# larskaislaniemi/PyLamp

Hardware: AMD Instinct MI355X
Metric: stokes_heat_mic_cell_updates_per_s (higher is better)
Workload: dtype f64

## Files before the change

pylamp_amd/csrc/pl_mic.h:

```cpp
#pragma once
#include "pl_internal.h"

#define PL_MAX_SCATTER_FIELDS 8
#define PL_MAX_GATHER_FIELDS 8

#define PL_AVG_PRELOG 64
struct PlScatterArgs {
    long long n;
    const double* tz; const double* tx;
    int nf;
    const double* f[PL_MAX_SCATTER_FIELDS];
    int scheme[PL_MAX_SCATTER_FIELDS];
    double z0, hz, x0, hx;
    double rhz, rhx;
    const double* zc; const double* xc;
    int nz, nx;
    int row0, nrows, col0, ncols;
    double* wsum; double* cnt;
    double* acc[PL_MAX_SCATTER_FIELDS];
    const int* cell_start; int ncz, ncx;
    int crow0, ccol0;
    int stag_z, stag_x;
};

// ... 79 lines not shown
    int nz, nx;
    int row0, nrows, col0, ncols;
    const int* cell_start; int ncz, ncx, crow0, ccol0;
    double* accN; double* accC; double* accZ; double* accX;
    long long N;
    int* slow_count; int* slow_list; int slow_cap;
    int dbg;
};
#define PL_SCF_MAX 10
struct PlScatterFinalArgs {
    int nz, nx, nf;
    const double* acc[PL_SCF_MAX]; const double* den[PL_SCF_MAX]; int scheme[PL_SCF_MAX]; double* out[PL_SCF_MAX];
    long long acc_pitch, out_pitch, out_off;
};
int pl_scatter_cells_device(pl_ctx* ctx, PlScatterCellsArgs& a, int variant);
void pl_launch_scatter_finalize_multi(pl_ctx* ctx, const PlScatterFinalArgs& a);

__device__ inline void mic_axis_locate(const double* __restrict__ c, int n, double z, int& ie, double& a) {
    if (z < c[0]) {
        const double h = c[1] - c[0], f = floor((z - c[0]) / h);
        ie = (int)f; a = (z - (c[0] + f * h)) / h;
        return;
    }
    if (z > c[n - 1]) {
        const double h = c[n - 1] - c[n - 2], f = floor((z - c[n - 1]) / h);
        ie = n - 1 + (int)f; a = (z - (c[n - 1] + f * h)) / h;
        return;
    }
    int lo = 0, hi = n - 1;
    while (hi - lo > 1) { const int mid = (lo + hi) >> 1; if (c[mid] <= z) lo = mid; else hi = mid; }
// ... 12 lines not shown
```

pylamp_amd/csrc/pl_mic_cells.hip:

```cpp
#include "pl_internal.h"
#include "pl_mic.h"

#define SC_Q 4
#define SC_NL 16
#define SC_W (SC_NL - 2)
#ifndef SC_ROWS
#define SC_ROWS 32
#endif
#ifndef SC_CAP
#define SC_CAP 320
#endif
#define SC_CAPP (SC_CAP + SC_CAP / 16 + 2)
#ifndef SC_NB
#define SC_NB 2
#endif

__device__ inline int sc_pidx(int o) { return o + (o >> 4); }

template <int CTRL> __device__ inline double sc_dpp(double v) {
    int lo = __double2loint(v), hi = __double2hiint(v);
    lo = __builtin_amdgcn_update_dpp(0, lo, CTRL, 0xf, 0xf, false);
    hi = __builtin_amdgcn_update_dpp(0, hi, CTRL, 0xf, 0xf, false);
    return __hiloint2double(hi, lo);
}
// ... 315 lines not shown
                const int di = cnr & 1, dj = cnr >> 1;
                double w = (dj ? cb : 1.0 - cb) * (di ? ca : 1.0 - ca);
                const bool flat = set == 1 && CEN == 2;
                if (flat) w = 1.0;
                add(base, ie + di, je + dj, w);
                for (int f = 0; f < nfs; f++) {
                    const int fk = set == 0 ? f : (NFN > 1 ? 1 : 0);
                    const double v = set <= 1 ? a.fn[fk][(IMASK >> fk) & 1u ? e : t] : a.fm[IND ? e : t];
                    add(base + (long long)(1 + f) * a.N, ie + di, je + dj, v * w);
                }
            }
        }
    }
}

__global__ __launch_bounds__(256) void k_scatter_finalize_multi(PlScatterFinalArgs a) {
    const int j = blockIdx.x * 64 + threadIdx.x, i = blockIdx.y * 4 + threadIdx.y;
    if (j >= a.nx || i >= a.nz) return;
    const long long o = (long long)i * a.acc_pitch + j, oo = a.out_off + (long long)i * a.out_pitch + j;
    for (int k = 0; k < a.nf; k++) {
        double s = a.acc[k][o];
        const double d = a.den[k][o];
        double r;
        if (a.scheme[k] & PL_AVG_ARITHMETIC) r = s / d;
        else { if (isinf(s)) s = 0.0; r = exp(s / d); }
        a.out[k][oo] = r;
    }
}

void pl_launch_scatter_finalize_multi(pl_ctx* ctx, const PlScatterFinalArgs& a) {
// ... 25 lines not shown
```

pylamp_amd/csrc/pl_step.hip:

```cpp
#include "pl_internal.h"
#include "pl_mic.h"
#include <algorithm>
#include <chrono>
#include <cmath>
#include <limits>

#define NFTRAC 13
enum { TR_RHO = 0, TR_ETA, TR_MRK, TR_TMP, TR_HCD, TR_HCP, TR_RH0, TR_ALP, TR_MAT, TR_ACE, TR_ET0, TR_IHT, TR__ID };
#define GASR 8.31446
#define PL_EPS (1.0 / 1024.0)

constexpr int X0_HIST = 5;
struct PlStepState {
    long long n = 0, cap = 0;
    double* tz = nullptr; double* tx = nullptr;
    double* tz2 = nullptr; double* tx2 = nullptr;
    double* f[NFTRAC] = {nullptr};
    double* vtz = nullptr; double* vtx = nullptr;
    double* tmp[3] = {nullptr, nullptr, nullptr};
    double* partial = nullptr;
    std::vector<double> hpartial;
    double* gcoords = nullptr;
    bool have_newtemp = false, have_solution = false, have_dT = false;
    int n_prev = 0;
    double* x_hist[X0_HIST] = {};
    double dt_hist[X0_HIST + 1] = {};
    double* f2[NFTRAC] = {nullptr};
    int* cell = nullptr; int* dest = nullptr;
    int* orig = nullptr; int* orig2 = nullptr;
    int* cell_count = nullptr; int* cell_start = nullptr; int* block_sums = nullptr;
    int ncz = 0, ncx = 0;
    int crow0 = 0, ccol0 = 0;
    bool sorted = false;
    int* need = nullptr; int* need_off = nullptr;
    int* need_flag = nullptr; int* need_rank = nullptr;
    int* cell_res = nullptr;
    double max_id = -1.0;
    bool max_id_valid = false;
    int sort_cells = 0;
    int* slot = nullptr; int* slot2 = nullptr;
    bool epoch_on = false; int epoch_age = 0;
    long long epoch_len = 0;
    bool lazy_pending = false, lazy_inject = false; long long lazy_n = 0;
    bool cols_undefined = false;
    std::vector<double> gmz, gmx;
    double* flags = nullptr; double* counts_dev = nullptr; int counts_cap = 0;
};

static PlStepState* state_of(pl_ctx* ctx) {
    if (!ctx->step) ctx->step = new PlStepState();
    return (PlStepState*)ctx->step;
}

void pl_step_free(pl_ctx* ctx) {
    PlStepState* s = (PlStepState*)ctx->step;
    if (!s) return;
    for (double* q : {s->tz, s->tx, s->tz2, s->tx2, s->vtz, s->vtx, s->tmp[0], s->tmp[1], s->tmp[2], s->partial, s->gcoords})
        if (q) (void)hipFree(q);
    for (double* q : s->f) if (q) (void)hipFree(q);
    for (double* q : s->f2) if (q) (void)hipFree(q);
    for (double* q : {s->flags, s->counts_dev}) if (q) (void)hipFree(q);
    for (int* q : {s->slot, s->slot2, s->cell, s->dest, s->orig, s->orig2, s->cell_count, s->cell_start, s->block_sums, s->need, s->need_off, s->need_flag, s->need_rank, s->cell_res}) if (q) (void)hipFree(q);
    delete s;
    ctx->step = nullptr;
}

static dim3 grid2d(const PlGeom& g) { return dim3((g.lnx + 63) / 64, (g.lnz + 3) / 4); }
static dim3 grid1d(long long n) { return dim3((unsigned)std::max<long long>((n + 255) / 256, 1)); }

__global__ __launch_bounds__(256) void k_soa_from_aos2(long long m, const double* __restrict__ src, double* __restrict__ a,
                                                       double* __restrict__ b) {
    long long t = (long long)blockIdx.x * blockDim.x + threadIdx.x;
    if (t < m) { a[t] = src[2 * t]; b[t] = src[2 * t + 1]; }
}
__global__ __launch_bounds__(256) void k_aos2_from_soa(long long m, const double* __restrict__ a, const double* __restrict__ b,
                                                       double* __restrict__ dst) {
    long long t = (long long)blockIdx.x * blockDim.x + threadIdx.x;
// ... 43 lines not shown
    const int base = blockIdx.x * 1024 + threadIdx.x * 4;
    int v[4], s = 0;
    for (int k = 0; k < 4; k++) { v[k] = (base + k < m) ? in[base + k] : 0; s += v[k]; }
    sh[threadIdx.x] = s;
    __syncthreads();
    for (int o = 1; o < 256; o <<= 1) {
        int add = (threadIdx.x >= o) ? sh[threadIdx.x - o] : 0;
        __syncthreads();
        sh[threadIdx.x] += add;
        __syncthreads();
    }
    int run = sh[threadIdx.x] - s;
    for (int k = 0; k < 4; k++) { if (base + k < m) out[base + k] = run; run += v[k]; }
    if (threadIdx.x == 255) bsum[blockIdx.x] = sh[255];
}
__global__ void k_scan_sums(int nb, int* __restrict__ bsum) {
    __shared__ int carry;
    if (threadIdx.x == 0) carry = 0;
    __syncthreads();
    for (int b0 = 0; b0 < nb; b0 += 256) {
        __shared__ int sh[256];
        const int k = b0 + threadIdx.x;
        const int v = (k < nb) ? bsum[k] : 0;
        sh[threadIdx.x] = v;
        __syncthreads();
        for (int o = 1; o < 256; o <<= 1) {
            int add = (threadIdx.x >= o) ? sh[threadIdx.x - o] : 0;
            __syncthreads();
            sh[threadIdx.x] += add;
            __syncthreads();
        }
        if (k < nb) bsum[k] = carry + sh[threadIdx.x] - v;
        __syncthreads();
        if (threadIdx.x == 255) carry += sh[255];
        __syncthreads();
    }
}
__global__ __launch_bounds__(256) void k_scan_add(int m, int* __restrict__ out, const int* __restrict__ bsum, int total_slot) {
    const int k = blockIdx.x * 256 + threadIdx.x;
    if (k < m) out[k] += bsum[k / 1024];
    (void)total_slot;
}
__global__ __launch_bounds__(256) void k_cell_place(long long n, const int* __restrict__ cell, const int* __restrict__ start,
                                                    int* __restrict__ fill, int* __restrict__ dest) {
    const long long t = (long long)blockIdx.x * blockDim.x + threadIdx.x;
    const int lane = threadIdx.x & 63;
    const int c = (t < n) ? cell[t] : -1;
    int seg0, len;
    mic_wave_runs(c, lane, seg0, len);
    int base = 0;
// ... 38 lines not shown
    const long long t = (long long)blockIdx.x * blockDim.x + threadIdx.x;
    const int lane = threadIdx.x & 63;
    const int c = (t < n) ? cell[t] : -1;
    int seg0, len;
    mic_wave_runs(c, lane, seg0, len);
    int base = 0;
    if (lane == seg0 && c >= 0) base = atomicAdd(&fill[c], len);
    base = __shfl(base, seg0, 64);
    if (c < 0) return;
    const int d = start[c] + base + (lane - seg0);
    dest[t] = d;
    for (int k = 0; k < a.na; k++) a.out[k][d] = a.in[k][t];
    slot_out[d] = slot_in ? slot_in[t] : (int)t;
}

__global__ __launch_bounds__(256) void k_deficit(int nc, int ncx, int row_lo, int row_hi, const int* __restrict__ start,
                                                 int dens, int dmin, int* __restrict__ need, int* __restrict__ flag) {
    const int c = blockIdx.x * 256 + threadIdx.x;
    if (c > nc) return;
    int v = 0;
    if (c < nc) {
        const int row = c / ncx;
        const int cnt = start[c + 1] - start[c];
        if (row >= row_lo && row < row_hi && cnt < dmin) v = dens - cnt;
    }
    need[c] = v;
    flag[c] = v > 0 ? 1 : 0;
}
__global__ __launch_bounds__(256) void k_max1d(long long n, const double* __restrict__ v, double* __restrict__ part) {
    double m = -INFINITY;
    for (long long t = (long long)blockIdx.x * 256 + threadIdx.x; t < n; t += (long long)gridDim.x * 256) m = fmax(m, v[t]);
    __shared__ double sh[4];
    for (int o = 32; o > 0; o >>= 1) m = fmax(m, __shfl_down(m, o, 64));
    if ((threadIdx.x & 63) == 0) sh[threadIdx.x >> 6] = m;
    __syncthreads();
    if (threadIdx.x == 0) part[blockIdx.x] = fmax(fmax(sh[0], sh[1]), fmax(sh[2], sh[3]));
}
__global__ __launch_bounds__(256) void k_mark_alive(long long n, const int* __restrict__ orig, int* __restrict__ alive) {
    const long long t = (long long)blockIdx.x * blockDim.x + threadIdx.x;
    if (t < n) alive[orig[t]] = 1;
}
__global__ __launch_bounds__(256) void k_remap_orig(long long n, int* __restrict__ orig, const int* __restrict__ rank) {
// ... 211 lines not shown
        *p = nullptr;
        PL_HIP(ctx, hipMalloc((void**)p, (size_t)cap * sizeof(double)));
        return 0;
    };
    for (double** q : {&S->tz, &S->tx, &S->tz2, &S->tx2, &S->vtz, &S->vtx, &S->tmp[0], &S->tmp[1], &S->tmp[2]}) PL_TRY(re(q));
    for (int k = 0; k < NFTRAC; k++) { PL_TRY(re(&S->f[k])); PL_TRY(re(&S->f2[k])); }
    for (int** q : {&S->cell, &S->dest, &S->orig, &S->orig2, &S->slot, &S->slot2}) {
        if (*q) (void)hipFree(*q);
        PL_HIP(ctx, hipMalloc((void**)q, (size_t)cap * sizeof(int)));
    }
    S->cap = cap;
    return 0;
}

static void unpermute(pl_ctx* ctx, PlStepState* S, int na, const double* const* in, double* const* out);
static bool scatter_cells_on() { const char* e = getenv("PYLAMP_SCATTER"); return !(e && atoi(e) == 0); }
static int ensure_current(pl_ctx* ctx, PlStepState* S);
struct SortOpts {
    bool full = false;
    int del_outside = 0; double Lz = 0.0, Lx = 0.0; long long* removed = nullptr;
    const pl_step_config* inject = nullptr; int it = 0; int64_t* ninjected = nullptr;
    bool keys_ready = false;
    bool premigrated = false;
    bool drop_trash = false;
};
static int sort_tracers(pl_ctx* ctx, PlStepState* S, double z0, double hz, double x0, double hx, const SortOpts& o = SortOpts());
static int ensure_coords(pl_ctx* ctx, PlStepState* S) {
    if (S->gcoords) return 0;
    if (S->gmz.empty()) {
        for (int d = 0; d < 2; d++) {
// ... 132 lines not shown
    }
    for (long long t0 = 0; t0 < n; t0 += chunk) {
        long long m = std::min<long long>(chunk, n - t0);
        hipLaunchKernelGGL(k_aos2_from_soa, grid1d(m), dim3(256), 0, ctx->stream, m, S->tz2 + t0, S->tx2 + t0, ctx->stage);
        PL_HIP(ctx, hipMemcpyAsync(out + 2 * t0, ctx->stage, (size_t)m * 2 * sizeof(double), hipMemcpyDeviceToHost, ctx->stream));
        PL_HIP(ctx, hipStreamSynchronize(ctx->stream));
    }
    return 0;
}

struct InjectSorted {
    int nc, ncx, crow0, ccol0;
    const int* start;
    const int* count;
    const int* need; const int* off; const int* rank;
    double* tz; double* tx; double* f[NFTRAC]; double* vtz; double* vtx; int* orig;
    double z0, hz, x0, hx; unsigned long long seed; unsigned step; double id0; int n_old;
    const double* zc; const double* xc;
    int* slot;
    int lazy;
};
__host__ __device__ inline bool tracer_const(int k) { return !(k == TR_RHO || k == TR_ETA || k == TR_TMP); }
__global__ __launch_bounds__(64) void k_inject_sorted(InjectSorted a) {
    const int c = blockIdx.x * 64 + threadIdx.x;
    if (c >= a.nc) return;
    const int m = a.need[c];
    if (m <= 0) return;
    const int t0 = a.start[c], t1 = t0 + a.count[c];
    const int ci = c / a.ncx + a.crow0, cj = c % a.ncx + a.ccol0;
    double mean[NFTRAC];
    for (int k = 0; k < NFTRAC; k++) {
        double sum = 0.0;
        if (a.lazy && (k == TR_RHO || k == TR_ETA)) { mean[k] = 0.0; continue; }
        if (a.slot && tracer_const(k)) for (int t = t0; t < t1; t++) sum += a.f[k][a.slot[t]];
        else for (int t = t0; t < t1; t++) sum += a.f[k][t];
        mean[k] = sum / (double)(t1 - t0);
    }
    for (int q = 0; q < m; q++) {
        const int d = t1 + q;
        const int e = a.slot ? a.n_old + a.off[c] + q : d;
        const unsigned gc = (unsigned)(ci * 65536 + cj);
        const double uz = inj_uniform(a.seed, gc, (unsigned)q, 2 * a.step), ux = inj_uniform(a.seed, gc, (unsigned)q, 2 * a.step + 1);
        a.tz[d] = a.zc ? a.zc[ci] + uz * (a.zc[ci + 1] - a.zc[ci]) : a.z0 + (ci + uz) * a.hz;
        a.tx[d] = a.xc ? a.xc[cj] + ux * (a.xc[cj + 1] - a.xc[cj]) : a.x0 + (cj + ux) * a.hx;
        for (int k = 0; k < NFTRAC; k++) {
            if (a.lazy && (k == TR_RHO || k == TR_ETA)) continue;
            a.f[k][tracer_const(k) ? e : d] = mean[k];
        }
        a.f[TR__ID][e] = a.id0 + a.off[c] + q - (a.rank ? a.rank[c] : 0);
        a.vtz[d] = 0.0; a.vtx[d] = 0.0;
        a.orig[e] = a.n_old + a.off[c] + q;
        if (a.slot) a.slot[d] = e;
    }
}
__global__ __launch_bounds__(64) void k_inject_fix_lazy(int nc, const int* __restrict__ start, const int* __restrict__ count,
                                                        const int* __restrict__ need, double* __restrict__ rho, double* __restrict__ eta) {
    const int c = blockIdx.x * 64 + threadIdx.x;
    if (c >= nc) return;
    const int m = need[c];
    if (m <= 0) return;
    const int t0 = start[c], t1 = t0 + count[c];
    double sr = 0.0, se = 0.0;
    for (int t = t0; t < t1; t++) sr += rho[t];
    for (int t = t0; t < t1; t++) se += eta[t];
    sr /= (double)(t1 - t0); se /= (double)(t1 - t0);
    for (int q = 0; q < m; q++) { rho[t1 + q] = sr; eta[t1 + q] = se; }
}
struct GatherColsArgs { const double* in[5]; double* out[5]; int na; };
__global__ __launch_bounds__(256) void k_gather_cols(long long n, const int* __restrict__ idx, GatherColsArgs a) {
    long long t = (long long)blockIdx.x * blockDim.x + threadIdx.x;
    if (t >= n) return;
    const int s = idx[t];
    for (int k = 0; k < a.na; k++) a.out[k][t] = a.in[k][s];
}
__global__ __launch_bounds__(256) void k_gather_int(long long n, const int* __restrict__ idx, const int* __restrict__ in, int* __restrict__ out) {
    long long t = (long long)blockIdx.x * blockDim.x + threadIdx.x;
    if (t < n) out[t] = in[idx[t]];
}
__global__ __launch_bounds__(256) void k_add_need(int nc, int m, const int* __restrict__ count, const int* __restrict__ need, int* __restrict__ total) {
    const int c = blockIdx.x * 256 + threadIdx.x;
    if (c < m) total[c] = count[c] + (c < nc ? need[c] : 0);
}

static int scan_ints(pl_ctx* ctx, PlStepState* S, int m, const int* in, int* out) {
    const int nb = (m + 1023) / 1024;
    hipLaunchKernelGGL(k_scan_block, dim3(nb), dim3(256), 0, ctx->stream, m, in, out, S->block_sums);
    hipLaunchKernelGGL(k_scan_sums, dim3(1), dim3(256), 0, ctx->stream, nb, S->block_sums);
    hipLaunchKernelGGL(k_scan_add, dim3((m + 255) / 256), dim3(256), 0, ctx->stream, m, out, S->block_sums, 0);
    return 0;
}

static int epoch_length() { const char* e = getenv("PYLAMP_EPOCH"); return e ? atoi(e) : 64; }
static int flush_lazy(pl_ctx* ctx, PlStepState* S) {
    if (!S->lazy_pending) return 0;
    S->lazy_pending = false;
    if (S->lazy_n > 0) {
        PermArgs pa{}; pa.na = 4;
        pa.in[0] = S->f2[TR_RHO]; pa.out[0] = S->f[TR_RHO]; pa.in[1] = S->f2[TR_ETA]; pa.out[1] = S->f[TR_ETA];
        pa.in[2] = S->tmp[0]; pa.out[2] = S->vtz; pa.in[3] = S->tmp[1]; pa.out[3] = S->vtx;
        hipLaunchKernelGGL(k_permute, grid1d(S->lazy_n), dim3(256), 0, ctx->stream, S->lazy_n, S->dest, pa);
    }
    if (S->lazy_inject)
        hipLaunchKernelGGL(k_inject_fix_lazy, dim3((S->sort_cells + 63) / 64), dim3(64), 0, ctx->stream, S->sort_cells, S->cell_start, S->cell_res,
                           S->need, S->f[TR_RHO], S->f[TR_ETA]);
    PL_HIP(ctx, hipGetLastError());
    return 0;
}
static int relayout(pl_ctx* ctx, PlStepState* S) {
    if (!S->epoch_on) return 0;
    S->epoch_on = false; S->epoch_age = 0;
    const long long n = S->n;
    if (n <= 0) return 0;
    int cols[NFTRAC], nc = 0;
    for (int k = 0; k < NFTRAC; k++) if (tracer_const(k)) cols[nc++] = k;
    for (int k0 = 0; k0 < nc; k0 += 5) {
        GatherColsArgs ga{}; ga.na = std::min(5, nc - k0);
        for (int k = 0; k < ga.na; k++) { ga.in[k] = S->f[cols[k0 + k]]; ga.out[k] = S->f2[cols[k0 + k]]; }
        hipLaunchKernelGGL(k_gather_cols, grid1d(n), dim3(256), 0, ctx->stream, n, S->slot, ga);
    }
// ... 16 lines not shown
    const PlGeom& g = ctx->geom.d;
    const int ncz = (g.gi0 + g.lnz >= g.nz) ? g.lnz - 1 : g.lnz;
    const int ncx = (g.gj0 + g.lnx >= g.nx) ? g.lnx - 1 : g.lnx;
    const int nc = ncz * ncx, m = nc + 10;
    S->crow0 = g.gi0; S->ccol0 = g.gj0;
    long long n = S->n;
    if (n >= (1LL << 31)) return pl_fail(ctx, "sort_tracers: more than 2^31 tracers per GPU");
    const bool epoch_ok = !o.full && epoch_length() > 0 && (ctx->nranks == 1 || o.premigrated) && !o.del_outside && ctx->geom.uniform && scatter_cells_on();
    if (!epoch_ok) PL_TRY(ensure_current(ctx, S));
    else {
        PL_TRY(flush_lazy(ctx, S));
        if (S->epoch_on && S->epoch_age >= epoch_length()) PL_TRY(relayout(ctx, S));
    }
    if (!S->cell_count || S->ncz != ncz || S->ncx != ncx) {
        if (o.keys_ready) return pl_fail(ctx, "sort_tracers: sort keys announced for another sort grid (internal error)");
        for (int** q : {&S->cell_count, &S->cell_start, &S->block_sums, &S->need, &S->need_off, &S->need_flag, &S->need_rank, &S->cell_res}) {
            if (*q) (void)hipFree(*q);
            *q = nullptr;
        }
        const int nb = (m + 1023) / 1024;
        for (int** q : {&S->cell_count, &S->cell_start, &S->need, &S->need_off, &S->need_flag, &S->need_rank, &S->cell_res})
            PL_HIP(ctx, hipMalloc((void**)q, (size_t)m * sizeof(int)));
        PL_HIP(ctx, hipMalloc((void**)&S->block_sums, (size_t)(nb + 1) * sizeof(int)));
        S->ncz = ncz; S->ncx = ncx;
    }
    S->sort_cells = nc;
    if (!o.keys_ready) {
        PL_HIP(ctx, hipMemsetAsync(S->cell_count, 0, (size_t)m * sizeof(int), ctx->stream));
        hipLaunchKernelGGL(k_cell_count, grid1d(n), dim3(256), 0, ctx->stream, n, S->tz, S->tx, z0, hz, x0, hx, coords_z(ctx, S, 0),
                           coords_x(ctx, S, 0), ncz, ncx, S->crow0, S->ccol0, g.nz - 1, g.nx - 1, S->cell, S->cell_count, o.del_outside, o.Lz, o.Lx);
    }
    long long ninj = 0; int ndef = 0;
    double id0 = 0.0; bool strict = false;
    const bool inj = o.inject && o.inject->tracdens_min > 0 && o.inject->tracdens > 0;
    if (inj) {
        const pl_step_config* cfg = o.inject;
        scan_ints(ctx, S, m, S->cell_count, S->cell_res);
        hipLaunchKernelGGL(k_deficit, dim3((nc + 1 + 255) / 256), dim3(256), 0, ctx->stream, nc, ncx, 0, ncz, S->cell_res, cfg->tracdens,
                           cfg->tracdens_min, S->need, S->need_flag);
        scan_ints(ctx, S, nc + 1, S->need, S->need_off);
        scan_ints(ctx, S, nc + 1, S->need_flag, S->need_rank);
        int h2[2] = {0, 0};
        PL_HIP(ctx, hipMemcpyAsync(&h2[0], S->need_off + nc, sizeof(int), hipMemcpyDeviceToHost, ctx->stream));
        PL_HIP(ctx, hipMemcpyAsync(&h2[1], S->need_rank + nc, sizeof(int), hipMemcpyDeviceToHost, ctx->stream));
        PL_HIP(ctx, hipStreamSynchronize(ctx->stream));
        ninj = h2[0]; ndef = h2[1];
        const int R = ctx->nranks;
        std::vector<double> cnt((size_t)2 * R, 0.0);
        cnt[2 * ctx->rank] = (double)ninj; cnt[2 * ctx->rank + 1] = ndef;
        if (R > 1) {
            PL_TRY(step_counts(ctx, S, 2 * R));
            hipLaunchKernelGGL(k_counts_from_ints, dim3(1), dim3(64), 0, ctx->stream, 1, (const int*)(S->need_off + nc), 0, S->counts_dev, 2 * ctx->rank);
            hipLaunchKernelGGL(k_counts_from_ints, dim3(1), dim3(64), 0, ctx->stream, 1, (const int*)(S->need_rank + nc), 0, S->counts_dev, 2 * ctx->rank + 1);
            PL_TRY(pl_comm_allreduce_dev(ctx, S->counts_dev, 2 * R, 0));
            PL_HIP(ctx, hipMemcpyAsync(cnt.data(), S->counts_dev, cnt.size() * sizeof(double), hipMemcpyDeviceToHost, ctx->stream));
            PL_HIP(ctx, hipStreamSynchronize(ctx->stream));
// ... 18 lines not shown
                    PL_HIP(ctx, hipStreamSynchronize(ctx->stream));
                    for (int k = 0; k < nbm; k++) mx[0] = std::fmax(mx[0], S->hpartial[k]);
                }
                PL_TRY(pl_allreduce_host(ctx, mx, 1, 2));
                S->max_id = mx[0]; S->max_id_valid = true;
            }
            strict = cfg->inject_unique_ids == 0;
            id0 = strict ? S->max_id + before - def_before : S->max_id + 1.0 + before;
            S->max_id += strict ? total - def_total : total;
        }
        if (ninj > 0) {
            const long long used = std::max(n, (epoch_ok && S->epoch_on) ? S->epoch_len : n);
            PL_TRY(grow_tracers(ctx, S, used + ninj, used));
        }
    }
    if (ninj > 0) {
        hipLaunchKernelGGL(k_add_need, dim3((m + 255) / 256), dim3(256), 0, ctx->stream, nc, m, S->cell_count, S->need, S->cell_res);
        scan_ints(ctx, S, m, S->cell_res, S->cell_start);
        PL_HIP(ctx, hipMemcpyAsync(S->cell_res, S->cell_count, (size_t)m * sizeof(int), hipMemcpyDeviceToDevice, ctx->stream));
    } else {
        scan_ints(ctx, S, m, S->cell_count, S->cell_start);
    }
    PL_HIP(ctx, hipMemsetAsync(S->cell_count, 0, (size_t)m * sizeof(int), ctx->stream));
    if (n > 0 && epoch_ok) {
        PermArgs pa{}; pa.na = 3;
        pa.in[0] = S->tz; pa.out[0] = S->tz2; pa.in[1] = S->tx; pa.out[1] = S->tx2; pa.in[2] = S->f[TR_TMP]; pa.out[2] = S->f2[TR_TMP];
        hipLaunchKernelGGL(k_place_permute, grid1d(n), dim3(256), 0, ctx->stream, n, S->cell, S->cell_start, S->cell_count, S->dest, pa,
                           S->epoch_on ? (const int*)S->slot : (const int*)nullptr, S->slot2);
        std::swap(S->tz, S->tz2); std::swap(S->tx, S->tx2);
        std::swap(S->vtz, S->tmp[0]); std::swap(S->vtx, S->tmp[1]);
        std::swap(S->slot, S->slot2);
        for (int k : {(int)TR_TMP, (int)TR_RHO, (int)TR_ETA}) std::swap(S->f[k], S->f2[k]);
    } else if (n > 0) {
        hipLaunchKernelGGL(k_cell_place, grid1d(n), dim3(256), 0, ctx->stream, n, S->cell, S->cell_start, S->cell_count, S->dest);
        const double* src[17]; double* dst[17];
        src[0] = S->tz; dst[0] = S->tz2; src[1] = S->tx; dst[1] = S->tx2;
// ... 6 lines not shown
        }
        hipLaunchKernelGGL(k_permute_int, grid1d(n), dim3(256), 0, ctx->stream, n, S->dest, S->orig, S->orig2);
        std::swap(S->tz, S->tz2); std::swap(S->tx, S->tx2); std::swap(S->orig, S->orig2);
        std::swap(S->vtz, S->tmp[0]); std::swap(S->vtx, S->tmp[1]);
        for (int k = 0; k < NFTRAC; k++) std::swap(S->f[k], S->f2[k]);
    }
    if (epoch_ok) {
        if (!S->epoch_on) S->epoch_len = n;
        S->epoch_age = S->epoch_on ? S->epoch_age + 1 : 1; S->epoch_on = true;
        S->lazy_pending = true; S->lazy_n = n; S->lazy_inject = ninj > 0;
    }
    if (ninj > 0) {
        InjectSorted a{};
        a.nc = nc; a.ncx = ncx; a.crow0 = S->crow0; a.ccol0 = S->ccol0; a.start = S->cell_start; a.count = S->cell_res;
        a.need = S->need; a.off = S->need_off; a.rank = strict ? S->need_rank : nullptr;
        a.tz = S->tz; a.tx = S->tx; for (int k = 0; k < NFTRAC; k++) a.f[k] = S->f[k];
        a.vtz = S->vtz; a.vtx = S->vtx; a.orig = S->orig;
        a.slot = epoch_ok ? S->slot : nullptr; a.lazy = epoch_ok ? 1 : 0;
        a.z0 = z0; a.hz = hz; a.x0 = x0; a.hx = hx; a.seed = o.inject->inject_seed; a.step = (unsigned)o.it; a.id0 = id0;
        a.n_old = (int)(epoch_ok ? S->epoch_len : n);
        if (epoch_ok) S->epoch_len += ninj;
        a.zc = coords_z(ctx, S, 0); a.xc = coords_x(ctx, S, 0);
        hipLaunchKernelGGL(k_inject_sorted, dim3((nc + 63) / 64), dim3(64), 0, ctx->stream, a);
        S->n = n + ninj;
    }
    if (o.ninjected) *o.ninjected = ninj;
    PL_HIP(ctx, hipGetLastError());
    if (o.removed) *o.removed = 0;
    if (o.drop_trash) {
        int keep = 0;
        PL_HIP(ctx, hipMemcpyAsync(&keep, S->cell_start + nc + 8, sizeof(int), hipMemcpyDeviceToHost, ctx->stream));
        PL_HIP(ctx, hipStreamSynchronize(ctx->stream));
        S->n = keep;
    }
    if (o.del_outside && n > 0) {
        int h[2] = {0, 0};
        PL_HIP(ctx, hipMemcpyAsync(h, S->cell_start + nc + 8, 2 * sizeof(int), hipMemcpyDeviceToHost, ctx->stream));
        PL_HIP(ctx, hipStreamSynchronize(ctx->stream));
        const int alive_n = h[0], all_n = h[1];
        if (alive_n < all_n) {
            PL_HIP(ctx, hipMemsetAsync(S->cell, 0, (size_t)all_n * sizeof(int), ctx->stream));
            if (alive_n > 0) hipLaunchKernelGGL(k_mark_alive, grid1d(alive_n), dim3(256), 0, ctx->stream, (long long)alive_n, S->orig, S->cell);
            const int nbb = (all_n + 1023) / 1024;
            int* bs = nullptr;
            PL_HIP(ctx, hipMalloc((void**)&bs, (size_t)(nbb + 1) * sizeof(int)));
            hipLaunchKernelGGL(k_scan_block, dim3(nbb), dim3(256), 0, ctx->stream, all_n, S->cell, S->dest, bs);
            hipLaunchKernelGGL(k_scan_sums, dim3(1), dim3(256), 0, ctx->stream, nbb, bs);
            hipLaunchKernelGGL(k_scan_add, dim3((all_n + 255) / 256), dim3(256), 0, ctx->stream, all_n, S->dest, bs, 0);
            if (alive_n > 0) hipLaunchKernelGGL(k_remap_orig, grid1d(alive_n), dim3(256), 0, ctx->stream, (long long)alive_n, S->orig, S->dest);
            PL_HIP(ctx, hipStreamSynchronize(ctx->stream));
            (void)hipFree(bs);
            if (o.removed) *o.removed = all_n - alive_n;
            S->n = alive_n;
            S->max_id_valid = false;
        }
    }
    if (o.del_outside && ctx->nranks > 1) {
        double v[1] = {S->max_id_valid ? 0.0 : 1.0};
        PL_TRY(pl_allreduce_host(ctx, v, 1, 2));
        if (v[0] > 0.0) S->max_id_valid = false;
    }
    return 0;
// ... 312 lines not shown
    ga.defval = std::numeric_limits<double>::quiet_NaN(); ga.accumulate = 0; ga.n_outside = (unsigned long long*)cnt;
    ga.g.nz = nz; ga.g.nx = nx; ga.g.gz = S->gcoords; ga.g.gx = S->gcoords + nz;
    ga.g.zmin = ctx->geom.zc[0]; ga.g.xmin = ctx->geom.xc[0];
    ga.g.Lz = ctx->geom.zc[nz - 1] - ctx->geom.zc[0]; ga.g.Lx = ctx->geom.xc[nx - 1] - ctx->geom.xc[0];
    ga.g.rect = ctx->geom.uniform ? 0 : 1;
    ga.g.fast_uniform = ctx->geom.uniform ? 1 : 0;
    ga.g.pitch = g.pitch; ga.g.off = pl_idx(g, -g.gi0, -g.gj0);
    if (first) {
        ga.fields[0] = P.newT; ga.out[0] = S->f[TR_TMP];
        pl_launch_gather(ctx, ga);
    } else {
        hipLaunchKernelGGL(k_plane_sub, grid2d(g), dim3(64, 4), 0, ctx->stream, g, P.newT, P.T, P.dT);
        PL_TRY(pl_halo(ctx, g, P.dT, 1, g.plane));
        S->have_dT = true;
        const double inv2 = (2.0 / dx) * (2.0 / dx) + (2.0 / dz) * (2.0 / dz);
        const bool fuse = ga.g.fast_uniform && !ga.g.rect;
        ga.fields[0] = P.dT; ga.out[0] = S->tmp[0];
        if (fuse) {
            ga.epi = 1; ga.epi_subgrid = cfg->do_subgrid_heatdiff; ga.epi_T = S->f[TR_TMP]; ga.epi_hcp = S->f[TR_HCP];
            ga.epi_rho = S->f[TR_RHO]; ga.epi_hcd = S->f[TR_HCD]; ga.epi_inv2 = inv2; ga.epi_dt = tstep;
            ga.epi_Tsub = S->tmp[1]; ga.epi_dTs = S->tmp[2]; ga.epi_ix = ix;
        }
        pl_launch_gather(ctx, ga);
        if (!fuse)
            hipLaunchKernelGGL(k_subgrid_part1, grid1d(n), dim3(256), 0, ctx->stream, n, S->f[TR_TMP], S->tmp[0], S->f[TR_HCP],
                               S->f[TR_RHO], S->f[TR_HCD], inv2, tstep, cfg->do_subgrid_heatdiff, S->tmp[1], S->tmp[2], ix);
        if (cfg->do_subgrid_heatdiff) {
            if (scatter_cells_on() && ctx->geom.uniform) {
                const double* fn[1] = {S->tmp[2]}; double* out[1] = {P.sgc};
                PL_TRY(scatter_cells(ctx, S, 2, fn, nullptr, q.z0, q.hz, q.x0, q.hx, out));
// ... 422 lines not shown
```

Baseline: 186.3 million.

## Fuse temperature-to-tracer gather, subgrid diffusion and scatter into one cell kernel; streamline census scans

```diff
diff --git a/pylamp_amd/csrc/pl_mic.h b/pylamp_amd/csrc/pl_mic.h
--- a/pylamp_amd/csrc/pl_mic.h
+++ b/pylamp_amd/csrc/pl_mic.h
@@ -117,6 +117,20 @@
     long long acc_pitch, out_pitch, out_off;
 };
 int pl_scatter_cells_device(pl_ctx* ctx, PlScatterCellsArgs& a, int variant);
+struct PlT2tCellsArgs {
+    const double* tz; const double* tx;
+    const double* T; double* Tout;
+    const double* rho; const double* hcp; const double* hcd;
+    const int* ix;
+    const double* dT; long long pitch, off;
+    const double* gz; const double* gx; double sz, sx;
+    double z0, hz, rhz, x0, hx, rhx;
+    double inv2, dt;
+    const int* cell_start; int ncz, ncx, crow0, ccol0;
+    long long n;
+    unsigned long long* counters;
+};
+int pl_t2t_cells_device(pl_ctx* ctx, PlT2tCellsArgs& a);
 void pl_launch_scatter_finalize_multi(pl_ctx* ctx, const PlScatterFinalArgs& a);
 
 __device__ inline void mic_axis_locate(const double* __restrict__ c, int n, double z, int& ie, double& a) {
diff --git a/pylamp_amd/csrc/pl_mic_cells.hip b/pylamp_amd/csrc/pl_mic_cells.hip
--- a/pylamp_amd/csrc/pl_mic_cells.hip
+++ b/pylamp_amd/csrc/pl_mic_cells.hip
@@ -353,6 +353,179 @@
     }
 }
 
+#define T2_ROWS 32
+template <bool IND>
+__global__ __launch_bounds__(64) void k_t2t_cells(PlT2tCellsArgs a, int strips_x) {
+    __shared__ double st[2][3][SC_CAPP];
+    __shared__ double ef[SC_CAPP];
+    __shared__ int kcol[2][SC_CAPP];
+    __shared__ int csl[T2_ROWS + 2][SC_NL + 1];
+    __shared__ double sgl[2][SC_NL], gxl[SC_NL], car[2][SC_NL];
+    __shared__ int ixs[IND ? SC_CAP : 1];
+    const int lane = threadIdx.x, q = lane >> 4, L = lane & 15;
+    const int sx = blockIdx.x % strips_x, sy = blockIdx.x / strips_x;
+    const int c0 = sx * SC_W, r0 = sy * T2_ROWS, r1 = min(r0 + T2_ROWS, a.ncz);
+    const int cc = c0 + L - 1;
+    const bool real = cc >= 0 && cc < a.ncx;
+    const int gj = a.ccol0 + cc;
+    const int nown = min(SC_W, a.ncx - c0);
+    const int i0 = max(r0 - 1, 0), i1 = min(r1 + 1, a.ncz);
+    const int cfirst = max(c0 - 1, 0), clast = min(c0 + SC_W + 1, a.ncx);
+    for (int k = lane; k < (i1 - i0) * (SC_NL + 1); k += 64) {
+        const int r = k / (SC_NL + 1), c = k % (SC_NL + 1);
+        const int col = min(max(c0 - 1 + c, cfirst), clast);
+        csl[r][c] = a.cell_start[(long long)(i0 + r) * a.ncx + col];
+    }
+    if (blockIdx.x == 0 && lane == 0 && (long long)a.cell_start[(long long)a.ncz * a.ncx] != a.n) atomicAdd(a.counters + 2, 1ull);
+    const double xc = a.x0 + gj * a.hx;
+    const double gxc = real ? a.gx[gj] : 0.0;
+    if (q == 0) { car[0][L] = 0.0; car[1][L] = 0.0; gxl[L] = gxc; }
+    __syncthreads();
+    constexpr int NU = SC_CAP / 64;
+    double pf[NU][6];
+    int pix[NU];
+    double dn0 = 0.0, dn1 = 0.0, dc0 = 0.0, dc1 = 0.0;
+    auto prefetch = [&](int row) {
+        const int b0 = csl[row - i0][0], b1 = min(b0 + SC_CAP, csl[row - i0][SC_NL]);
+#pragma unroll
+        for (int u = 0; u < NU; u++) {
+            const int t = b0 + lane + 64 * u;
+            if (t < b1) {
+                const int e = IND ? ixs[lane + 64 * u] : t;
+                pf[u][0] = a.tz[t]; pf[u][1] = a.tx[t]; pf[u][2] = a.T[t]; pf[u][3] = a.rho[t]; pf[u][4] = a.hcp[e]; pf[u][5] = a.hcd[e];
+            }
+        }
+        if (real) {
+            const long long o = a.off + (long long)(a.crow0 + row + 1) * a.pitch + gj;
+            dn0 = a.dT[o]; dn1 = a.dT[o + 1];
+        }
+        if (IND && row + 1 < i1) {
+            const int c0n = csl[row + 1 - i0][0], c1n = min(c0n + SC_CAP, csl[row + 1 - i0][SC_NL]);
+#pragma unroll
+            for (int u = 0; u < NU; u++) { const int t = c0n + lane + 64 * u; if (t < c1n) pix[u] = a.ix[t]; }
+        }
+    };
+    auto phase_b = [&](int j) {
+        const int pj = j & 1;
+        const int b0 = csl[j - i0][0], b1 = min(b0 + SC_CAP, csl[j - i0][SC_NL]);
+        const double gzj = a.gz[a.crow0 + j];
+#pragma unroll
+        for (int u = 0; u < NU; u++) {
+            const int t = b0 + lane + 64 * u;
+            if (t >= b1) continue;
+            const int o = sc_pidx(t - b0);
+            const int Lc = kcol[pj][o];
+            if (Lc < 1 || Lc > nown) continue;
+            const double z = st[pj][0][o], x = st[pj][1][o], ts = st[pj][2][o];
+            const double ca = (z - gzj) * a.sz, cb = (x - gxl[Lc]) * a.sx;
+            const double v = (1 - cb) * (1 - ca) * sgl[pj][Lc] + cb * (1 - ca) * sgl[pj][Lc + 1] + (1 - cb) * ca * sgl[pj ^ 1][Lc] +
+                             cb * ca * sgl[pj ^ 1][Lc + 1];
+            a.Tout[t] = ts - v;
+        }
+    };
+    if (i0 < i1) {
+        if (IND) {
+            const int b0 = csl[0][0], b1 = min(b0 + SC_CAP, csl[0][SC_NL]);
+#pragma unroll
+            for (int u = 0; u < NU; u++) { const int t = b0 + lane + 64 * u; if (t < b1) ixs[lane + 64 * u] = a.ix[t]; }
+            __syncthreads();
+        }
+        if (real) {
+            const long long o = a.off + (long long)(a.crow0 + i0) * a.pitch + gj;
+            dc0 = a.dT[o]; dc1 = a.dT[o + 1];
+        }
+        prefetch(i0);
+    }
+    for (int i = i0; i < i1; i++) {
+        const int gi = a.crow0 + i, par = i & 1;
+        const double zc = a.z0 + gi * a.hz;
+        const double gzi = a.gz[gi];
+        const int wrow0 = csl[i - i0][0], wrow1 = csl[i - i0][SC_NL];
+        const int we = min(wrow0 + SC_CAP, wrow1);
+        if (wrow1 - wrow0 > SC_CAP && lane == 0) atomicAdd(a.counters + 2, 1ull);
+        int s = 0, e = 0;
+        if (real) { s = csl[i - i0][L]; e = csl[i - i0][L + 1]; }
+        const double d00 = dc0, d01 = dc1, d10 = dn0, d11 = dn1;
+        dc0 = dn0; dc1 = dn1;
+#pragma unroll
+        for (int u = 0; u < NU; u++) {
+            const int t = wrow0 + lane + 64 * u;
+            if (t < we) {
+                const int o = sc_pidx(t - wrow0);
+                st[par][0][o] = pf[u][0]; st[par][1][o] = pf[u][1]; st[par][2][o] = pf[u][2];
+                const double dt0 = pf[u][4] * pf[u][3] / (pf[u][5] * a.inv2);
+                ef[o] = exp(-0.5 * a.dt / dt0);
+            }
+        }
+        if (IND && i + 1 < i1) {
+            const int c0n = csl[i + 1 - i0][0], c1n = min(c0n + SC_CAP, csl[i + 1 - i0][SC_NL]);
+#pragma unroll
+            for (int u = 0; u < NU; u++) if (c0n + lane + 64 * u < c1n) ixs[lane + 64 * u] = pix[u];
+        }
+        __syncthreads();
+        if (i + 1 < i1) prefetch(i + 1);
+        double N[2][2][2];
+#pragma unroll
+        for (int di = 0; di < 2; di++)
+#pragma unroll
+            for (int dj = 0; dj < 2; dj++) { N[di][dj][0] = 0.0; N[di][dj][1] = 0.0; }
+        const int tend = min(e, we);
+        for (int t = s + q; t < tend; t += SC_Q) {
+            const int o = sc_pidx(t - wrow0);
+            const double z = st[par][0][o], x = st[par][1][o];
+            const double ca = (z - zc) * a.rhz, cb = (x - xc) * a.rhx;
+            if (!(ca >= 0.0 && ca < 1.0 && cb >= 0.0 && cb < 1.0)) {
+                if (L >= 1 && L <= nown && i >= r0 && i < r1) atomicAdd(a.counters + 1, 1ull);
+                kcol[par][o] = -1;
+                continue;
+            }
+            const double ga = (z - gzi) * a.sz, gb = (x - gxc) * a.sx;
+            const double v = (1 - gb) * (1 - ga) * d00 + gb * (1 - ga) * d01 + (1 - gb) * ga * d10 + gb * ga * d11;
+            const double Told = st[par][2][o], Tnew = Told + v;
+            const double ts = Told - (Told - Tnew) * ef[o];
+            const double f = ts - Tnew;
+            st[par][2][o] = ts; kcol[par][o] = L;
+            const double wz2[2] = {1.0 - ca, ca}, wx2[2] = {1.0 - cb, cb};
+#pragma unroll
+            for (int di = 0; di < 2; di++)
+#pragma unroll
+                for (int dj = 0; dj < 2; dj++) {
+                    const double w = wx2[dj] * wz2[di];
+                    N[di][dj][0] += w;
+                    N[di][dj][1] += f * w;
+                }
+        }
+        double Hn[2][2];
+#pragma unroll
+        for (int di = 0; di < 2; di++)
+#pragma unroll
+            for (int k = 0; k < 2; k++) Hn[di][k] = sc_qsum(N[di][0][k] + sc_left(N[di][1][k]));
+        if (q == 0) {
+            const double den = Hn[0][0] + car[0][L], num = Hn[0][1] + car[1][L];
+            car[0][L] = Hn[1][0]; car[1][L] = Hn[1][1];
+            sgl[par][L] = num / den;
+        }
+        __syncthreads();
+        if (i - 1 >= r0 && i - 1 < r1) phase_b(i - 1);
+        __syncthreads();
+    }
+    if (i1 > i0 && i1 - 1 >= r0 && i1 - 1 < r1) {
+        if (q == 0) sgl[i1 & 1][L] = car[1][L] / car[0][L];
+        __syncthreads();
+        phase_b(i1 - 1);
+    }
+}
+
+int pl_t2t_cells_device(pl_ctx* ctx, PlT2tCellsArgs& a) {
+    if (a.ncz <= 0 || a.ncx <= 0) return 0;
+    a.rhz = 1.0 / a.hz; a.rhx = 1.0 / a.hx;
+    const int strips_x = (a.ncx + SC_W - 1) / SC_W, strips_z = (a.ncz + T2_ROWS - 1) / T2_ROWS;
+    if (a.ix) hipLaunchKernelGGL((k_t2t_cells<true>), dim3((unsigned)(strips_x * strips_z)), dim3(64), 0, ctx->stream, a, strips_x);
+    else hipLaunchKernelGGL((k_t2t_cells<false>), dim3((unsigned)(strips_x * strips_z)), dim3(64), 0, ctx->stream, a, strips_x);
+    PL_HIP(ctx, hipGetLastError());
+    return 0;
+}
+
 __global__ __launch_bounds__(256) void k_scatter_finalize_multi(PlScatterFinalArgs a) {
     const int j = blockIdx.x * 64 + threadIdx.x, i = blockIdx.y * 4 + threadIdx.y;
     if (j >= a.nx || i >= a.nz) return;
diff --git a/pylamp_amd/csrc/pl_step.hip b/pylamp_amd/csrc/pl_step.hip
--- a/pylamp_amd/csrc/pl_step.hip
+++ b/pylamp_amd/csrc/pl_step.hip
@@ -33,7 +33,8 @@
     int crow0 = 0, ccol0 = 0;
     bool sorted = false;
     int* need = nullptr; int* need_off = nullptr;
-    int* need_flag = nullptr; int* need_rank = nullptr;
+    int* need_list = nullptr; int* need_rank = nullptr;
+    int need_cells = 0;
     int* cell_res = nullptr;
     double max_id = -1.0;
     bool max_id_valid = false;
@@ -60,7 +61,7 @@
     for (double* q : s->f) if (q) (void)hipFree(q);
     for (double* q : s->f2) if (q) (void)hipFree(q);
     for (double* q : {s->flags, s->counts_dev}) if (q) (void)hipFree(q);
-    for (int* q : {s->slot, s->slot2, s->cell, s->dest, s->orig, s->orig2, s->cell_count, s->cell_start, s->block_sums, s->need, s->need_off, s->need_flag, s->need_rank, s->cell_res}) if (q) (void)hipFree(q);
+    for (int* q : {s->slot, s->slot2, s->cell, s->dest, s->orig, s->orig2, s->cell_count, s->cell_start, s->block_sums, s->need, s->need_off, s->need_list, s->need_rank, s->cell_res}) if (q) (void)hipFree(q);
     delete s;
     ctx->step = nullptr;
 }
@@ -134,26 +135,27 @@
     for (int k = 0; k < 4; k++) { if (base + k < m) out[base + k] = run; run += v[k]; }
     if (threadIdx.x == 255) bsum[blockIdx.x] = sh[255];
 }
-__global__ void k_scan_sums(int nb, int* __restrict__ bsum) {
-    __shared__ int carry;
-    if (threadIdx.x == 0) carry = 0;
+template <int NA>
+__global__ __launch_bounds__(1024) void k_scan_sums(int nb, int* __restrict__ bsum, int ns) {
+    __shared__ int sh[NA][1024];
+    const int per = (nb + 1023) / 1024, k0 = min(threadIdx.x * per, nb), k1 = min(k0 + per, nb);
+    int s[NA];
+    for (int a = 0; a < NA; a++) {
+        s[a] = 0;
+        for (int k = k0; k < k1; k++) s[a] += bsum[(size_t)a * ns + k];
+        sh[a][threadIdx.x] = s[a];
+    }
     __syncthreads();
-    for (int b0 = 0; b0 < nb; b0 += 256) {
-        __shared__ int sh[256];
-        const int k = b0 + threadIdx.x;
-        const int v = (k < nb) ? bsum[k] : 0;
-        sh[threadIdx.x] = v;
+    for (int o = 1; o < 1024; o <<= 1) {
+        int add[NA];
+        for (int a = 0; a < NA; a++) add[a] = (threadIdx.x >= o) ? sh[a][threadIdx.x - o] : 0;
         __syncthreads();
-        for (int o = 1; o < 256; o <<= 1) {
-            int add = (threadIdx.x >= o) ? sh[threadIdx.x - o] : 0;
-            __syncthreads();
-            sh[threadIdx.x] += add;
-            __syncthreads();
-        }
-        if (k < nb) bsum[k] = carry + sh[threadIdx.x] - v;
+        for (int a = 0; a < NA; a++) sh[a][threadIdx.x] += add[a];
         __syncthreads();
-        if (threadIdx.x == 255) carry += sh[255];
-        __syncthreads();
+    }
+    for (int a = 0; a < NA; a++) {
+        int run = sh[a][threadIdx.x] - s[a];
+        for (int k = k0; k < k1; k++) { const int v = bsum[(size_t)a * ns + k]; bsum[(size_t)a * ns + k] = run; run += v; }
     }
 }
 __global__ __launch_bounds__(256) void k_scan_add(int m, int* __restrict__ out, const int* __restrict__ bsum, int total_slot) {
@@ -222,18 +224,59 @@
     slot_out[d] = slot_in ? slot_in[t] : (int)t;
 }
 
-__global__ __launch_bounds__(256) void k_deficit(int nc, int ncx, int row_lo, int row_hi, const int* __restrict__ start,
-                                                 int dens, int dmin, int* __restrict__ need, int* __restrict__ flag) {
+struct CensusScan {
+    int m, nc, dens, dmin;
+    const int* count;
+    int* start; int* need; int* off; int* rank;
+    int* res;
+    int* list;
+    int* bsum; int ns;
+};
+template <bool INJ>
+__global__ __launch_bounds__(256) void k_census_block(CensusScan a) {
+    constexpr int NA = INJ ? 3 : 1;
+    __shared__ int sh[NA][256];
+    const int base = blockIdx.x * 1024 + threadIdx.x * 4;
+    int cnt[4], nd[4], s[3] = {0, 0, 0};
+    for (int k = 0; k < 4; k++) {
+        const int c = base + k;
+        cnt[k] = (c < a.m) ? a.count[c] : 0;
+        nd[k] = (INJ && c < a.nc && cnt[k] < a.dmin) ? a.dens - cnt[k] : 0;
+        s[0] += cnt[k] + nd[k]; s[1] += nd[k]; s[2] += nd[k] > 0 ? 1 : 0;
+    }
+    for (int q = 0; q < NA; q++) sh[q][threadIdx.x] = s[q];
+    __syncthreads();
+    for (int o = 1; o < 256; o <<= 1) {
+        int add[NA];
+        for (int q = 0; q < NA; q++) add[q] = (threadIdx.x >= o) ? sh[q][threadIdx.x - o] : 0;
+        __syncthreads();
+        for (int q = 0; q < NA; q++) sh[q][threadIdx.x] += add[q];
+        __syncthreads();
+    }
+    int run[3] = {0, 0, 0};
+    for (int q = 0; q < NA; q++) run[q] = sh[q][threadIdx.x] - s[q];
+    for (int k = 0; k < 4; k++) {
+        const int c = base + k;
+        if (c < a.m) {
+            a.start[c] = run[0];
+            if (INJ) { a.need[c] = nd[k]; a.off[c] = run[1]; a.rank[c] = run[2]; a.res[c] = cnt[k]; }
+        }
+        run[0] += cnt[k] + nd[k]; run[1] += nd[k]; run[2] += nd[k] > 0 ? 1 : 0;
+    }
+    if (threadIdx.x == 255) for (int q = 0; q < NA; q++) a.bsum[(size_t)q * a.ns + blockIdx.x] = sh[q][255];
+}
+template <bool INJ>
+__global__ __launch_bounds__(256) void k_census_add(CensusScan a) {
     const int c = blockIdx.x * 256 + threadIdx.x;
-    if (c > nc) return;
-    int v = 0;
-    if (c < nc) {
-        const int row = c / ncx;
-        const int cnt = start[c + 1] - start[c];
-        if (row >= row_lo && row < row_hi && cnt < dmin) v = dens - cnt;
-    }
-    need[c] = v;
-    flag[c] = v > 0 ? 1 : 0;
+    if (c >= a.m) return;
+    const int b = c / 1024;
+    a.start[c] += a.bsum[b];
+    if (INJ) {
+        a.off[c] += a.bsum[(size_t)a.ns + b];
+        const int r = a.rank[c] + a.bsum[(size_t)2 * a.ns + b];
+        a.rank[c] = r;
+        if (a.need[c] > 0) a.list[r] = c;
+    }
 }
 __global__ __launch_bounds__(256) void k_max1d(long long n, const double* __restrict__ v, double* __restrict__ part) {
     double m = -INFINITY;
@@ -475,6 +518,7 @@
 }
 
 static void unpermute(pl_ctx* ctx, PlStepState* S, int na, const double* const* in, double* const* out);
+static int t2t_mode() { const char* e = getenv("PYLAMP_T2T"); return e ? atoi(e) : 1; }
 static bool scatter_cells_on() { const char* e = getenv("PYLAMP_SCATTER"); return !(e && atoi(e) == 0); }
 static int ensure_current(pl_ctx* ctx, PlStepState* S);
 struct SortOpts {
@@ -637,6 +681,7 @@
     const int* start;
     const int* count;
     const int* need; const int* off; const int* rank;
+    const int* list; int ndef;
     double* tz; double* tx; double* f[NFTRAC]; double* vtz; double* vtx; int* orig;
     double z0, hz, x0, hx; unsigned long long seed; unsigned step; double id0; int n_old;
     const double* zc; const double* xc;
@@ -644,22 +689,30 @@
     int lazy;
 };
 __host__ __device__ inline bool tracer_const(int k) { return !(k == TR_RHO || k == TR_ETA || k == TR_TMP); }
+constexpr int INJ_LANES = 16, INJ_CELLS = 64 / INJ_LANES;
+static_assert(NFTRAC <= INJ_LANES, "one lane per field");
 __global__ __launch_bounds__(64) void k_inject_sorted(InjectSorted a) {
-    const int c = blockIdx.x * 64 + threadIdx.x;
-    if (c >= a.nc) return;
-    const int m = a.need[c];
-    if (m <= 0) return;
-    const int t0 = a.start[c], t1 = t0 + a.count[c];
+    __shared__ double mean[INJ_CELLS][NFTRAC];
+    const int grp = threadIdx.x / INJ_LANES, l = threadIdx.x % INJ_LANES;
+    const int i = blockIdx.x * INJ_CELLS + grp;
+    const int c = i < a.ndef ? a.list[i] : -1;
+    const int m = c >= 0 ? a.need[c] : 0;
+    const int t0 = c >= 0 ? a.start[c] : 0, t1 = c >= 0 ? t0 + a.count[c] : 0;
+    if (c >= 0 && l < NFTRAC) {
+        const int k = l;
+        double sum = 0.0;
+        if (a.lazy && (k == TR_RHO || k == TR_ETA)) mean[grp][k] = 0.0;
+        else {
+            const double* __restrict__ fk = a.f[k];
+            if (a.slot && tracer_const(k)) for (int t = t0; t < t1; t++) sum += fk[a.slot[t]];
+            else for (int t = t0; t < t1; t++) sum += fk[t];
+            mean[grp][k] = sum / (double)(t1 - t0);
+        }
+    }
+    __syncthreads();
+    if (c < 0) return;
     const int ci = c / a.ncx + a.crow0, cj = c % a.ncx + a.ccol0;
-    double mean[NFTRAC];
-    for (int k = 0; k < NFTRAC; k++) {
-        double sum = 0.0;
-        if (a.lazy && (k == TR_RHO || k == TR_ETA)) { mean[k] = 0.0; continue; }
-        if (a.slot && tracer_const(k)) for (int t = t0; t < t1; t++) sum += a.f[k][a.slot[t]];
-        else for (int t = t0; t < t1; t++) sum += a.f[k][t];
-        mean[k] = sum / (double)(t1 - t0);
-    }
-    for (int q = 0; q < m; q++) {
+    for (int q = l; q < m; q += INJ_LANES) {
         const int d = t1 + q;
         const int e = a.slot ? a.n_old + a.off[c] + q : d;
         const unsigned gc = (unsigned)(ci * 65536 + cj);
@@ -668,7 +721,7 @@
         a.tx[d] = a.xc ? a.xc[cj] + ux * (a.xc[cj + 1] - a.xc[cj]) : a.x0 + (cj + ux) * a.hx;
         for (int k = 0; k < NFTRAC; k++) {
             if (a.lazy && (k == TR_RHO || k == TR_ETA)) continue;
-            a.f[k][tracer_const(k) ? e : d] = mean[k];
+            a.f[k][tracer_const(k) ? e : d] = mean[grp][k];
         }
         a.f[TR__ID][e] = a.id0 + a.off[c] + q - (a.rank ? a.rank[c] : 0);
         a.vtz[d] = 0.0; a.vtx[d] = 0.0;
@@ -676,18 +729,23 @@
         if (a.slot) a.slot[d] = e;
     }
 }
-__global__ __launch_bounds__(64) void k_inject_fix_lazy(int nc, const int* __restrict__ start, const int* __restrict__ count,
-                                                        const int* __restrict__ need, double* __restrict__ rho, double* __restrict__ eta) {
-    const int c = blockIdx.x * 64 + threadIdx.x;
-    if (c >= nc) return;
-    const int m = need[c];
-    if (m <= 0) return;
-    const int t0 = start[c], t1 = t0 + count[c];
-    double sr = 0.0, se = 0.0;
-    for (int t = t0; t < t1; t++) sr += rho[t];
-    for (int t = t0; t < t1; t++) se += eta[t];
-    sr /= (double)(t1 - t0); se /= (double)(t1 - t0);
-    for (int q = 0; q < m; q++) { rho[t1 + q] = sr; eta[t1 + q] = se; }
+__global__ __launch_bounds__(64) void k_inject_fix_lazy(int ndef, const int* __restrict__ list, const int* __restrict__ start,
+                                                        const int* __restrict__ count, const int* __restrict__ need,
+                                                        double* __restrict__ rho, double* __restrict__ eta) {
+    __shared__ double mean[INJ_CELLS][2];
+    const int grp = threadIdx.x / INJ_LANES, l = threadIdx.x % INJ_LANES;
+    const int i = blockIdx.x * INJ_CELLS + grp;
+    const int c = i < ndef ? list[i] : -1;
+    const int m = c >= 0 ? need[c] : 0;
+    const int t0 = c >= 0 ? start[c] : 0, t1 = c >= 0 ? t0 + count[c] : 0;
+    if (c >= 0 && l < 2) {
+        const double* __restrict__ v = l == 0 ? rho : eta;
+        double sum = 0.0;
+        for (int t = t0; t < t1; t++) sum += v[t];
+        mean[grp][l] = sum / (double)(t1 - t0);
+    }
+    __syncthreads();
+    for (int q = l; q < m; q += INJ_LANES) { rho[t1 + q] = mean[grp][0]; eta[t1 + q] = mean[grp][1]; }
 }
 struct GatherColsArgs { const double* in[5]; double* out[5]; int na; };
 __global__ __launch_bounds__(256) void k_gather_cols(long long n, const int* __restrict__ idx, GatherColsArgs a) {
@@ -700,19 +758,6 @@
     long long t = (long long)blockIdx.x * blockDim.x + threadIdx.x;
     if (t < n) out[t] = in[idx[t]];
 }
-__global__ __launch_bounds__(256) void k_add_need(int nc, int m, const int* __restrict__ count, const int* __restrict__ need, int* __restrict__ total) {
-    const int c = blockIdx.x * 256 + threadIdx.x;
-    if (c < m) total[c] = count[c] + (c < nc ? need[c] : 0);
-}
-
-static int scan_ints(pl_ctx* ctx, PlStepState* S, int m, const int* in, int* out) {
-    const int nb = (m + 1023) / 1024;
-    hipLaunchKernelGGL(k_scan_block, dim3(nb), dim3(256), 0, ctx->stream, m, in, out, S->block_sums);
-    hipLaunchKernelGGL(k_scan_sums, dim3(1), dim3(256), 0, ctx->stream, nb, S->block_sums);
-    hipLaunchKernelGGL(k_scan_add, dim3((m + 255) / 256), dim3(256), 0, ctx->stream, m, out, S->block_sums, 0);
-    return 0;
-}
-
 static int epoch_length() { const char* e = getenv("PYLAMP_EPOCH"); return e ? atoi(e) : 64; }
 static int flush_lazy(pl_ctx* ctx, PlStepState* S) {
     if (!S->lazy_pending) return 0;
@@ -724,8 +769,8 @@
         hipLaunchKernelGGL(k_permute, grid1d(S->lazy_n), dim3(256), 0, ctx->stream, S->lazy_n, S->dest, pa);
     }
     if (S->lazy_inject)
-        hipLaunchKernelGGL(k_inject_fix_lazy, dim3((S->sort_cells + 63) / 64), dim3(64), 0, ctx->stream, S->sort_cells, S->cell_start, S->cell_res,
-                           S->need, S->f[TR_RHO], S->f[TR_ETA]);
+        hipLaunchKernelGGL(k_inject_fix_lazy, dim3((S->need_cells + INJ_CELLS - 1) / INJ_CELLS), dim3(64), 0, ctx->stream, S->need_cells, S->need_list,
+                           S->cell_start, S->cell_res, S->need, S->f[TR_RHO], S->f[TR_ETA]);
     PL_HIP(ctx, hipGetLastError());
     return 0;
 }
@@ -772,14 +817,14 @@
     }
     if (!S->cell_count || S->ncz != ncz || S->ncx != ncx) {
         if (o.keys_ready) return pl_fail(ctx, "sort_tracers: sort keys announced for another sort grid (internal error)");
-        for (int** q : {&S->cell_count, &S->cell_start, &S->block_sums, &S->need, &S->need_off, &S->need_flag, &S->need_rank, &S->cell_res}) {
+        for (int** q : {&S->cell_count, &S->cell_start, &S->block_sums, &S->need, &S->need_off, &S->need_list, &S->need_rank, &S->cell_res}) {
             if (*q) (void)hipFree(*q);
             *q = nullptr;
         }
         const int nb = (m + 1023) / 1024;
-        for (int** q : {&S->cell_count, &S->cell_start, &S->need, &S->need_off, &S->need_flag, &S->need_rank, &S->cell_res})
+        for (int** q : {&S->cell_count, &S->cell_start, &S->need, &S->need_off, &S->need_list, &S->need_rank, &S->cell_res})
             PL_HIP(ctx, hipMalloc((void**)q, (size_t)m * sizeof(int)));
-        PL_HIP(ctx, hipMalloc((void**)&S->block_sums, (size_t)(nb + 1) * sizeof(int)));
+        PL_HIP(ctx, hipMalloc((void**)&S->block_sums, (size_t)3 * nb * sizeof(int)));
         S->ncz = ncz; S->ncx = ncx;
     }
     S->sort_cells = nc;
@@ -791,13 +836,16 @@
     long long ninj = 0; int ndef = 0;
     double id0 = 0.0; bool strict = false;
     const bool inj = o.inject && o.inject->tracdens_min > 0 && o.inject->tracdens > 0;
+    const int nb = (m + 1023) / 1024;
+    CensusScan cs{};
+    cs.m = m; cs.nc = nc; cs.count = S->cell_count; cs.start = S->cell_start; cs.need = S->need; cs.off = S->need_off; cs.rank = S->need_rank;
+    cs.res = S->cell_res; cs.list = S->need_list; cs.bsum = S->block_sums; cs.ns = nb;
     if (inj) {
         const pl_step_config* cfg = o.inject;
-        scan_ints(ctx, S, m, S->cell_count, S->cell_res);
-        hipLaunchKernelGGL(k_deficit, dim3((nc + 1 + 255) / 256), dim3(256), 0, ctx->stream, nc, ncx, 0, ncz, S->cell_res, cfg->tracdens,
-                           cfg->tracdens_min, S->need, S->need_flag);
-        scan_ints(ctx, S, nc + 1, S->need, S->need_off);
-        scan_ints(ctx, S, nc + 1, S->need_flag, S->need_rank);
+        cs.dens = cfg->tracdens; cs.dmin = cfg->tracdens_min;
+        hipLaunchKernelGGL(k_census_block<true>, dim3(nb), dim3(256), 0, ctx->stream, cs);
+        hipLaunchKernelGGL(k_scan_sums<3>, dim3(1), dim3(1024), 0, ctx->stream, nb, S->block_sums, nb);
+        hipLaunchKernelGGL(k_census_add<true>, dim3((m + 255) / 256), dim3(256), 0, ctx->stream, cs);
         int h2[2] = {0, 0};
         PL_HIP(ctx, hipMemcpyAsync(&h2[0], S->need_off + nc, sizeof(int), hipMemcpyDeviceToHost, ctx->stream));
         PL_HIP(ctx, hipMemcpyAsync(&h2[1], S->need_rank + nc, sizeof(int), hipMemcpyDeviceToHost, ctx->stream));
@@ -846,12 +894,10 @@
             PL_TRY(grow_tracers(ctx, S, used + ninj, used));
         }
     }
-    if (ninj > 0) {
-        hipLaunchKernelGGL(k_add_need, dim3((m + 255) / 256), dim3(256), 0, ctx->stream, nc, m, S->cell_count, S->need, S->cell_res);
-        scan_ints(ctx, S, m, S->cell_res, S->cell_start);
-        PL_HIP(ctx, hipMemcpyAsync(S->cell_res, S->cell_count, (size_t)m * sizeof(int), hipMemcpyDeviceToDevice, ctx->stream));
-    } else {
-        scan_ints(ctx, S, m, S->cell_count, S->cell_start);
+    if (!inj) {
+        hipLaunchKernelGGL(k_census_block<false>, dim3(nb), dim3(256), 0, ctx->stream, cs);
+        hipLaunchKernelGGL(k_scan_sums<1>, dim3(1), dim3(1024), 0, ctx->stream, nb, S->block_sums, nb);
+        hipLaunchKernelGGL(k_census_add<false>, dim3((m + 255) / 256), dim3(256), 0, ctx->stream, cs);
     }
     PL_HIP(ctx, hipMemsetAsync(S->cell_count, 0, (size_t)m * sizeof(int), ctx->stream));
     if (n > 0 && epoch_ok) {
@@ -888,6 +934,7 @@
         InjectSorted a{};
         a.nc = nc; a.ncx = ncx; a.crow0 = S->crow0; a.ccol0 = S->ccol0; a.start = S->cell_start; a.count = S->cell_res;
         a.need = S->need; a.off = S->need_off; a.rank = strict ? S->need_rank : nullptr;
+        a.list = S->need_list; a.ndef = ndef; S->need_cells = ndef;
         a.tz = S->tz; a.tx = S->tx; for (int k = 0; k < NFTRAC; k++) a.f[k] = S->f[k];
         a.vtz = S->vtz; a.vtx = S->vtx; a.orig = S->orig;
         a.slot = epoch_ok ? S->slot : nullptr; a.lazy = epoch_ok ? 1 : 0;
@@ -895,7 +942,7 @@
         a.n_old = (int)(epoch_ok ? S->epoch_len : n);
         if (epoch_ok) S->epoch_len += ninj;
         a.zc = coords_z(ctx, S, 0); a.xc = coords_x(ctx, S, 0);
-        hipLaunchKernelGGL(k_inject_sorted, dim3((nc + 63) / 64), dim3(64), 0, ctx->stream, a);
+        hipLaunchKernelGGL(k_inject_sorted, dim3((ndef + INJ_CELLS - 1) / INJ_CELLS), dim3(64), 0, ctx->stream, a);
         S->n = n + ninj;
     }
     if (o.ninjected) *o.ninjected = ninj;
@@ -919,7 +966,7 @@
             int* bs = nullptr;
             PL_HIP(ctx, hipMalloc((void**)&bs, (size_t)(nbb + 1) * sizeof(int)));
             hipLaunchKernelGGL(k_scan_block, dim3(nbb), dim3(256), 0, ctx->stream, all_n, S->cell, S->dest, bs);
-            hipLaunchKernelGGL(k_scan_sums, dim3(1), dim3(256), 0, ctx->stream, nbb, bs);
+            hipLaunchKernelGGL(k_scan_sums<1>, dim3(1), dim3(1024), 0, ctx->stream, nbb, bs, nbb);
             hipLaunchKernelGGL(k_scan_add, dim3((all_n + 255) / 256), dim3(256), 0, ctx->stream, all_n, S->dest, bs, 0);
             if (alive_n > 0) hipLaunchKernelGGL(k_remap_orig, grid1d(alive_n), dim3(256), 0, ctx->stream, (long long)alive_n, S->orig, S->dest);
             PL_HIP(ctx, hipStreamSynchronize(ctx->stream));
@@ -1262,6 +1309,25 @@
         PL_TRY(pl_halo(ctx, g, P.dT, 1, g.plane));
         S->have_dT = true;
         const double inv2 = (2.0 / dx) * (2.0 / dx) + (2.0 / dz) * (2.0 / dz);
+        const int t2t = t2t_mode();
+        if (t2t != 0 && ctx->nranks == 1 && ctx->geom.uniform && scatter_cells_on() && cfg->do_subgrid_heatdiff && n > 0 && S->sorted) {
+            PlT2tCellsArgs ta{};
+            ta.tz = S->tz; ta.tx = S->tx; ta.T = S->f[TR_TMP]; ta.Tout = S->f2[TR_TMP];
+            ta.rho = S->f[TR_RHO]; ta.hcp = S->f[TR_HCP]; ta.hcd = S->f[TR_HCD]; ta.ix = ix;
+            ta.dT = P.dT; ta.pitch = ga.g.pitch; ta.off = ga.g.off;
+            ta.gz = ga.g.gz; ta.gx = ga.g.gx; ta.sz = (nz - 1) / ga.g.Lz; ta.sx = (nx - 1) / ga.g.Lx;
+            ta.z0 = q.z0; ta.hz = q.hz; ta.x0 = q.x0; ta.hx = q.hx; ta.inv2 = inv2; ta.dt = tstep;
+            ta.cell_start = S->cell_start; ta.ncz = S->ncz; ta.ncx = S->ncx; ta.crow0 = S->crow0; ta.ccol0 = S->ccol0;
+            ta.n = n; ta.counters = (unsigned long long*)cnt;
+            PL_TRY(pl_t2t_cells_device(ctx, ta));
+            unsigned long long h[3] = {0, 0, 0};
+            PL_HIP(ctx, hipMemcpyAsync(h, cnt, sizeof(h), hipMemcpyDeviceToHost, ctx->stream));
+            PL_HIP(ctx, hipStreamSynchronize(ctx->stream));
+            if (h[1] == 0 && h[2] == 0 && t2t != 2) { std::swap(S->f[TR_TMP], S->f2[TR_TMP]); return 0; }
+            if (getenv("PYLAMP_T2T_LOG"))
+                fprintf(stderr, "pylamp: temp_to_tracers takes the three-pass path (%llu tracers outside their sorted cell, %llu strip rows beyond the window)\n",
+                        h[1], h[2]);
+        }
         const bool fuse = ga.g.fast_uniform && !ga.g.rect;
         ga.fields[0] = P.dT; ga.out[0] = S->tmp[0];
         if (fuse) {
```

Result: slower. 173.4 million (-6.9%).
